# pariasm/bwd-nlkalman

Hardware: AMD Instinct MI355X
Metric: Mpix/s per frame (nlkalman-flt, 1080p sigma=20) (higher is better)
Workload: dtype f32; 1 GPU; C2: 1920x1080x3 synthetic AWGN sigma=20, FLT1 temporal (deno0 = spatial FLT1 of frame 0, bsic1=NULL), patch 8, defaults of nlkalman_default_params; parallelism=single GPU, mask_order=serial-exact, match_order=exact (the reference's hy, hx, c order)

## Files before the change

bwd-nlkalman_amd/csrc/k_frame.h:

```cpp
#pragma once
#include "nlk_common.h"

template <int CH>
__global__ void __launch_bounds__(256)
k_layout(const float* __restrict__ cur, float* __restrict__ pl_cur, const float* __restrict__ prev,
         float* __restrict__ pl_prev, const float* __restrict__ basic, float* __restrict__ pl_basic,
         uint8_t* __restrict__ rowok, float* __restrict__ acc_zero, int w, int h, int ch, int psz, int planar,
         int y0,
         uint32_t* __restrict__ zero_word,
         float* __restrict__ pl_diff) {
  const int x = blockIdx.x * blockDim.x + threadIdx.x, y = y0 + blockIdx.y;
  if (zero_word && x == 0 && blockIdx.y == 0) *zero_word = 0u;
  if (x >= w) return;
  const size_t npix = (size_t)w * h, i = (size_t)y * w + x;
  float own = 0.f;
  if constexpr (CH == 3) {
    struct __attribute__((packed, aligned(4))) P3 { float v[3]; };
    const P3 a = reinterpret_cast<const P3*>(cur)[i];
    P3 b = a, d = a;
    if (prev) b = reinterpret_cast<const P3*>(prev)[i];
    if (basic) d = reinterpret_cast<const P3*>(basic)[i];
    own = b.v[0];
#pragma unroll
    for (int c = 0; c < 3; ++c) {
      pl_cur[c * npix + i] = a.v[c];
      if (prev) pl_prev[c * npix + i] = b.v[c];
      if (basic) pl_basic[c * npix + i] = d.v[c];
      if (pl_diff) pl_diff[c * npix + i] = b.v[c] - a.v[c];
    }
  } else {
    if (prev) own = prev[i * ch];
    if (planar) {
      for (int c = 0; c < ch; ++c) {
        pl_cur[c * npix + i] = cur[i * ch + c];
        if (prev) pl_prev[c * npix + i] = prev[i * ch + c];
        if (basic) pl_basic[c * npix + i] = basic[i * ch + c];
        if (pl_diff) pl_diff[c * npix + i] = prev[i * ch + c] - cur[i * ch + c];
      }
    }
  }
  if (prev) {
#ifdef NLK_LAYOUT_ROWOK_LOADS
    uint8_t ok = (x + psz <= w);
    if (ok)
      for (int j = 0; j < psz; ++j) {
        const float v = prev[(i + j) * ch];
        if (v != v) ok = 0;
      }
    rowok[i] = ok;
#else
    const int lane = threadIdx.x & 63;
    const int xh = x + 64;
    const bool halo_nan = lane < psz - 1 && xh < w && prev[((size_t)y * w + xh) * ch] != prev[((size_t)y * w + xh) * ch];
    const uint64_t m_lo = __ballot(own != own), m_hi = __ballot(halo_nan);
    const uint64_t win = (m_lo >> lane) | (lane ? m_hi << (64 - lane) : 0ull);
    rowok[i] = (x + psz <= w) && (win & ((1ull << psz) - 1ull)) == 0ull;
#endif
  }
  if (acc_zero)
    for (int c = 0; c <= ch; ++c) acc_zero[c * npix + i] = 0.f;
}

__global__ void k_nan_cols(const uint8_t* __restrict__ rowok, uint8_t* __restrict__ valid,
                           int w, int h, int psz, int y0) {
  const int x = blockIdx.x * blockDim.x + threadIdx.x, y = y0 + blockIdx.y;
  if (x >= w) return;
  uint8_t ok = (y + psz <= h);
  if (ok)
    for (int i = 0; i < psz; ++i) ok &= rowok[(size_t)(y + i) * w + x];
  valid[(size_t)y * w + x] = ok;
}
__global__ void k_nan_cols4(const uint32_t* __restrict__ rowok, uint32_t* __restrict__ valid,
                            int w4, int h, int psz, int y0) {
  const int x = blockIdx.x * blockDim.x + threadIdx.x, y = y0 + blockIdx.y;
  if (x >= w4) return;
  uint32_t ok = (y + psz <= h) ? 0x01010101u : 0u;
  if (ok)
    for (int i = 0; i < psz; ++i) ok &= rowok[(size_t)(y + i) * w4 + x];
  valid[(size_t)y * w4 + x] = ok;
}

template <int CH>
__global__ void k_normalize(float* __restrict__ out, const float* __restrict__ acc,
                            const float* __restrict__ cur_hwc, int w, int h, int ch,
                            int y0, int y1) {
  const size_t npix = (size_t)w * h;
  for (size_t i = (size_t)y0 * w + blockIdx.x * blockDim.x + threadIdx.x;
       i < (size_t)y1 * w; i += (size_t)gridDim.x * blockDim.x) {
    if constexpr (CH == 3) {
      struct __attribute__((packed, aligned(4))) P3 { float v[3]; };
      const float a = acc[(size_t)3 * npix + i];
      P3 o;
      if (a > 1e-6f) {
#pragma unroll
        for (int c = 0; c < 3; ++c) o.v[c] = acc[(size_t)c * npix + i] / a;
      } else {
        o = reinterpret_cast<const P3*>(cur_hwc)[i];
      }
      reinterpret_cast<P3*>(out)[i] = o;
    } else {
      const float a = acc[(size_t)ch * npix + i];
      for (int c = 0; c < ch; ++c)
        out[i * ch + c] = a > 1e-6f ? acc[(size_t)c * npix + i] / a : cur_hwc[i * ch + c];
    }
  }
}

__global__ void k_add(float* __restrict__ dst, const float* __restrict__ src, size_t n) {
  for (size_t i = blockIdx.x * (size_t)blockDim.x + threadIdx.x; i < n; i += (size_t)gridDim.x * blockDim.x)
    dst[i] += src[i];
}

__global__ void k_rgb2opp(float* __restrict__ im, size_t npix) {
  const float a = 1.f / sqrtf(3.f), b = 1.f / sqrtf(2.f);
  const float c = 2.f * a * sqrtf(2.f);
  for (size_t i = blockIdx.x * (size_t)blockDim.x + threadIdx.x; i < npix;
       i += (size_t)gridDim.x * blockDim.x) {
    float* p = im + 3 * i;
    const float r = p[0], g = p[1], bl = p[2];
    p[0] = a * (r + g + bl);
// ... 85 lines not shown
```

bwd-nlkalman_amd/csrc/k_group8m.h:

```cpp
#pragma once
#include "nlk_common.h"
#include "k_commit_rows.h"
#include "k_group8.h"
#include "k_group_math.h"
#include <type_traits>

typedef float nlk_f4 __attribute__((ext_vector_type(4)));

#define NLK_G8_SST 136
#ifndef NLK_G8_CW
#define NLK_G8_CW 16
#define NLK_G8_CH 4
#endif
static inline int nlk_g8m_grid(int ntx, int nty) {
  const int nch = ((ntx + NLK_G8_CW - 1) / NLK_G8_CW) * ((nty + NLK_G8_CH - 1) / NLK_G8_CH);
  return ((nch + 7) / 8) * 8 * NLK_G8_CW * NLK_G8_CH;
}

__device__ __forceinline__ float nlk_bperm(float v, int src_lane) {
  return __int_as_float(__builtin_amdgcn_ds_bpermute(src_lane << 2, __float_as_int(v)));
}
__device__ __forceinline__ uint32_t nlk_bperm_u(uint32_t v, int src_lane) {
  return (uint32_t)__builtin_amdgcn_ds_bpermute(src_lane << 2, (int)v);
}
// ... 407 lines not shown
          constexpr bool s5_add = MODE == 1;
#endif
#pragma unroll
          for (int j = 0; j < 2; ++j) {
            const float mk = (float)((mbyte >> (2 * g4 + j)) & 1u);
#pragma unroll
            for (int q = 0; q < 4; ++q) {
              const float di = C[q][j], d = C[q][j + 2];
              if (MODE == 2) {
                S[0][q] += di;
                S[1][q] = fmaf(di, di, S[1][q]);
              }
              S[2][q] += d;
              S[3][q] = fmaf(d, d, S[3][q]);
              const float df = di - d;
              if (MODE == 2) S[4][q] = fmaf(mk * df, df, S[4][q]);
              else S[4][q] = fmaf(df, df, S[4][q]);
            }
          }
          if (s5_add) {
#pragma unroll
            for (int j = 0; j < 2; ++j) {
              const float mk = (float)((mbyte >> (2 * g4 + j)) & 1u);
#pragma unroll
              for (int q = 0; q < 4; ++q) S[5][q] = fmaf(mk, C[q][j + 2], S[5][q]);
            }
          }
        } else {
#pragma unroll
          for (int j = 0; j < 4; ++j)
#pragma unroll
            for (int q = 0; q < 4; ++q) {
              S[0][q] += C[q][j];
              S[1][q] = fmaf(C[q][j], C[q][j], S[1][q]);
            }
        }
        if (b == nb - 1) {
#if NLK_G8_S5TRACK
          if (MODE == 1 && s5_track) {
#pragma unroll
            for (int q = 0; q < 4; ++q) S[5][q] = S[2][q];
          }
          s5_track = true;
#endif
          float T[6];
#pragma unroll
          for (int a = 0; a < 6; ++a) {
            T[a] = 0.f;
            const bool used = MODE == 0 ? a < 2 : (MODE == 1 ? a >= 2 : a < 5);
            if (used) {
              const auto x = __builtin_amdgcn_permlane32_swap(__float_as_uint(S[a][0]), __float_as_uint(S[a][2]), false, false);
              const auto y = __builtin_amdgcn_permlane32_swap(__float_as_uint(S[a][1]), __float_as_uint(S[a][3]), false, false);
              const float X = __uint_as_float(x[0]) + __uint_as_float(x[1]);
              const float Y = __uint_as_float(y[0]) + __uint_as_float(y[1]);
              const auto z = __builtin_amdgcn_permlane16_swap(__float_as_uint(X), __float_as_uint(Y), false, false);
              T[a] = __uint_as_float(z[0]) + __uint_as_float(z[1]);
            }
          }
          {
            const float nx0q = g4 == 0 ? NX0[0][0] : (g4 == 1 ? NX0[1][0] : (g4 == 2 ? NX0[2][0] : NX0[3][0]));
            const float v0 = (T[3] - T[2] * T[2] * in0) * in0;
            const float v01n = T[4] * in0;
            float a, term, m;
            const float v1 = (T[1] - T[0] * T[0] * in1) * in1;
            nlk_gain<MODE, true>(v1, v0, v01n, g, s2, a, term);
            m = MODE == 2 ? 0.f : (MODE == 1 ? T[5] * ing : T[0] * in1) - nx0q;
            part_sum += term;
            const int cidx = SEPB ? 16 * (lo & 3) + 4 * g4 + (lo >> 2) : 16 * g4 + lo;
            stash[ch * SST + cidx] = a;
            stash[ch * SST + 64 + cidx] = (1 - a) * m;
          }
#pragma unroll
          for (int a = 0; a < 6; ++a)
#pragma unroll
            for (int q = 0; q < 4; ++q) S[a][q] = 0.f;
        }
      }
    };
    if (np0 == 0) pass_a(std::integral_constant<int, 0>{});
    else if (!SMO) pass_a(std::integral_constant<int, 1>{});
    else pass_a(std::integral_constant<int, 2>{});
    } else {
    float* const x0buf = stash + NSLOT * SST;
    auto sep_gain = [&](auto mode_tag, const auto& T, int ch) {
      constexpr int MODE = decltype(mode_tag)::value;
      constexpr int NS = MODE == 0 ? 2 : (MODE == 1 ? 4 : 5);
        const int oq = 2 * ((lane >> 2) & 1) + (lane >> 5), oa = (lane >> 3) & 3;
        const float nx0q = x0buf[16 * si + 4 * oq + oa];
        const int cidx = SEPB ? 16 * si + 4 * oq + oa : 16 * oq + 4 * oa + si;
        float a, term, m;
        if (MODE == 2) {
          const float v1 = (T[1] - T[0] * T[0] * in1) * in1;
          const float v0 = (T[NS > 3 ? 3 : 0] - T[NS > 2 ? 2 : 0] * T[NS > 2 ? 2 : 0] * in0) * in0;
          nlk_gain<2, true>(v1, v0, T[NS > 4 ? 4 : 0] * in0, g, s2, a, term);
          m = 0.f;
        } else if (MODE == 1) {
          const float v0 = (T[1] - T[0] * T[0] * in0) * in0;
          nlk_gain<1, true>(0.f, v0, T[NS > 2 ? 2 : 0] * in0, g, s2, a, term);
          m = (T[0] - T[NS > 3 ? 3 : 0]) * ing - nx0q;
        } else {
          const float v1 = (T[1] - T[0] * T[0] * in1) * in1;
          nlk_gain<0, true>(v1, 0.f, 0.f, g, s2, a, term);
          m = T[0] * in1 - nx0q;
        }
        part_sum += term;
        stash[ch * SST + cidx] = a;
        stash[ch * SST + 64 + cidx] = (1 - a) * m;
    };
    auto pass_a = [&](auto mode_tag) {
      constexpr int MODE = decltype(mode_tag)::value;
      constexpr bool HP = MODE != 0;
      constexpr int NS = MODE == 0 ? 2 : (MODE == 1 ? 4 : 5);
      const int nb = (k + 7) >> 3;
      if (nb == 0) return;
      const int hh = (lane >> 2) & 1, hp = lane >> 3;
      const bool odd = (lane & 1) != 0;
      const uint32_t rowx = (uint32_t)(((lane & 6) * g.w + (odd ? 4 : 0)) * 4);
      const uint32_t rowy = (uint32_t)((((lane & 6) + 1) * g.w + (odd ? 0 : 4)) * 4);
      const float sgn = hh ? -1.f : 1.f;
      float sEh[4];
#pragma unroll
      for (int i = 0; i < 4; ++i) sEh[i] = hh ? -sE[1][3 - i] : sE[0][i];
      const uint32_t e_dead = o_first + e_img;
      auto slot_offs = [&](int bb, uint32_t& oi, uint32_t& op) {
        const int ci = 8 * bb + hp, cl = min(ci, k - 1);
        const uint32_t oc = nlk_bperm_u(cl < 64 ? oreg[0] : oreg[1], cl & 63);
        const bool in_k = ci < k, valid = (oc >> 31) != 0u;
        const uint32_t o = oc & 0x7fffffffu;
        const bool live_i = MODE == 1 ? (in_k && valid) : in_k;
        oi = live_i ? o + e_img : e_dead;
        op = (in_k && valid) ? o + e_prev : e_dead;
      };
      int rows_seen = 0;
      auto row_read = [&](uint32_t off, int cc, float (&R)[8]) {
#ifdef NLK_G8_EXP_NOROWS
        if (rows_seen >= 2) { asm volatile("" : "+v"(R[0]), "+v"(R[3]), "+v"(R[5]), "+v"(R[7]) : "v"(off)); return; }
        ++rows_seen;
#endif
#ifdef NLK_G8_EXP_LDSROWS
        if (rows_seen >= 2) {
          const float* wp = smem + ((off + (uint32_t)cc * 7u + (uint32_t)(lane & 7) * 18u) % 1500u);
#pragma unroll
          for (int c = 0; c < 8; ++c) R[c] = wp[c];
          return;
        }
        ++rows_seen;
#endif
        typedef const __attribute__((address_space(1))) nlk_f4u* gp4;
        const char* bp = reinterpret_cast<const char*>(pbase);
        const uint32_t o = (off + (uint32_t)cc * (uint32_t)npix) * 4u;
        const nlk_f4u a0 = *(gp4)(bp + (size_t)(o + rowx)), a1 = *(gp4)(bp + (size_t)(o + rowy));
#pragma unroll
        for (int c = 0; c < 4; ++c) { R[c] = a0[c]; R[4 + c] = a1[c]; }
      };
      auto fold_half = [&](const float (&R)[8], float (&F)[2][4]) {
        float Z[4], S[4];
#pragma unroll
        for (int c = 0; c < 4; ++c) {
          Z[c] = odd ? R[4 + c] : R[c];
          S[c] = odd ? R[c] : R[4 + c];
        }
#pragma unroll
        for (int c = 0; c < 4; ++c) {
          const float rt = nlk_dpp<NLK_DPP_XOR1>(S[3 - c]);
          F[0][c] = Z[c] + rt;
          F[1][c] = Z[c] - rt;
        }
#define NLK_G8_FMAC_HM(i) "v_fmac_f32_dpp %" #i ", %" #i ", %8 row_half_mirror row_mask:0xf bank_mask:0xf bound_ctrl:1\n\t"
        asm("s_nop 1\n\t" NLK_G8_FMAC_HM(0) NLK_G8_FMAC_HM(1) NLK_G8_FMAC_HM(2) NLK_G8_FMAC_HM(3) NLK_G8_FMAC_HM(4)
            NLK_G8_FMAC_HM(5) NLK_G8_FMAC_HM(6) NLK_G8_FMAC_HM(7)
            : "+v"(F[0][0]), "+v"(F[0][1]), "+v"(F[0][2]), "+v"(F[0][3]), "+v"(F[1][0]), "+v"(F[1][1]), "+v"(F[1][2]),
              "+v"(F[1][3])
            : "v"(sgn));
#undef NLK_G8_FMAC_HM
      };
      auto fwd_half = [&](const float (&F)[2][4], nlk_f4 (&Y)[2]) {
        nlk_f4 T[2] = {nlk_f4{0.f, 0.f, 0.f, 0.f}, nlk_f4{0.f, 0.f, 0.f, 0.f}};
#pragma unroll
        for (int kk = 0; kk < 4; ++kk)
#pragma unroll
          for (int qc = 0; qc < 2; ++qc) T[qc] = nlk_mfma4(F[qc][kk], sE[qc][kk], T[qc]);
#pragma unroll
        for (int i = 0; i < 4; ++i)
#pragma unroll
          for (int qc = 0; qc < 2; ++qc) Y[qc] = nlk_mfma4(sEh[i], T[qc][i], Y[qc]);
      };
      nlk_f4* const x0w = reinterpret_cast<nlk_f4*>(x0buf + 16 * si + 8 * hh);
      const nlk_f4* const x0v = x0w;
      float S[NS][2][4];
#pragma unroll
      for (int a = 0; a < NS; ++a)
#pragma unroll
        for (int q = 0; q < 2; ++q)
#pragma unroll
          for (int j = 0; j < 4; ++j) S[a][q][j] = 0.f;
      float Ri[8], Rp[8];
      uint32_t oi, op, oin, opn;
      slot_offs(0, oi, op);
      const uint32_t oi0 = oi, op0 = op;
      row_read(oi, 0, Ri);
      if (HP) row_read(op, 0, Rp);
      slot_offs(1, oin, opn);
      for (int ch = 0; ch < CH; ++ch)
      for (int b = 0; b < nb; ++b) {
        const bool wrap = b + 1 == nb;
        const int chn = wrap ? min(ch + 1, CH - 1) : ch;
#ifdef NLK_G8_EXP_LDSROWS
        if (HP && b == 0) {
          float* win = stash + nlk_g8_stash_floats<CH, SEP>();
          const uint32_t back = 10u * (uint32_t)g.w + 10u;
          const uint32_t wo = (o_first > back ? o_first - back : o_first) + (uint32_t)ch * (uint32_t)npix;
          float tmp[12];
#pragma unroll
          for (int kq = 0; kq < 6; ++kq) {
            const uint32_t idx = min((uint32_t)lane + 64u * kq, 323u), r = (idx * 3641u) >> 16, cx = idx - 18u * r;
            tmp[kq] = pbase[(size_t)(e_img + wo + r * (uint32_t)g.w + cx)];
            tmp[6 + kq] = pbase[(size_t)(e_prev + wo + r * (uint32_t)g.w + cx)];
          }
#pragma unroll
          for (int kq = 0; kq < 6; ++kq) {
            win[(lane + 64 * kq) % (NLK_G8_LDS_PAD / 8)] = tmp[kq];
            win[NLK_G8_LDS_PAD / 8 + (lane + 64 * kq) % (NLK_G8_LDS_PAD / 8)] = tmp[6 + kq];
          }
          nlk_wave_lds_order();
        }
#endif
        float Fi[2][4], Fp[2][4];
        fold_half(Ri, Fi);
        if (HP) fold_half(Rp, Fp);
        uint32_t o_in = wrap ? oi0 : oin, o_pn = wrap ? op0 : opn;
        if (HP)
          asm volatile("" : "+v"(Fi[0][0]), "+v"(Fi[0][1]), "+v"(Fi[0][2]), "+v"(Fi[0][3]), "+v"(Fi[1][0]), "+v"(Fi[1][1]),
                       "+v"(Fi[1][2]), "+v"(Fi[1][3]), "+v"(Fp[0][0]), "+v"(Fp[0][1]), "+v"(Fp[0][2]), "+v"(Fp[0][3]),
                       "+v"(Fp[1][0]), "+v"(Fp[1][1]), "+v"(Fp[1][2]), "+v"(Fp[1][3]), "+v"(o_in), "+v"(o_pn));
        else
          asm volatile("" : "+v"(Fi[0][0]), "+v"(Fi[0][1]), "+v"(Fi[0][2]), "+v"(Fi[0][3]), "+v"(Fi[1][0]), "+v"(Fi[1][1]),
                       "+v"(Fi[1][2]), "+v"(Fi[1][3]), "+v"(o_in));
        __builtin_amdgcn_sched_barrier(0);
        row_read(o_in, chn, Ri);
        if (HP) row_read(o_pn, chn, Rp);
        __builtin_amdgcn_sched_barrier(0);
        slot_offs(wrap ? 1 : b + 2, oin, opn);
        nlk_f4 Yi[2], Yp[2];
        if (b == 0) {
          Yi[0] = Yi[1] = nlk_f4{0.f, 0.f, 0.f, 0.f};
          fwd_half(Fi, Yi);
          if (hp == 0) { x0w[0] = -Yi[0]; x0w[1] = -Yi[1]; }
          nlk_wave_lds_order();
          Yi[0] += x0v[0]; Yi[1] += x0v[1];
        } else {
          Yi[0] = x0v[0]; Yi[1] = x0v[1];
          fwd_half(Fi, Yi);
        }
        if (HP) {
          Yp[0] = x0v[0]; Yp[1] = x0v[1];
          fwd_half(Fp, Yp);
        }
        if constexpr (HP) {
          const uint64_t vw = b < 8 ? vbits[0] : vbits[1], gw = b < 8 ? gbits[0] : gbits[1];
          const uint32_t vch = (uint32_t)(vw >> (8 * (b & 7))) & 0xffu, gch = (uint32_t)(gw >> (8 * (b & 7))) & 0xffu;
          if constexpr (MODE == 1) {
            const bool mixed = (vch & ~gch) != 0u;
            const float mkc = (float)((~gch >> hp) & 1u);
#pragma unroll
            for (int q = 0; q < 2; ++q)
#pragma unroll
              for (int j = 0; j < 4; ++j) {
                const float di = Yi[q][j], d = Yp[q][j];
                const float df = di - d;
                if (b == 0) {
                  S[0][q][j] = d;
                  S[1][q][j] = d * d;
                  S[2][q][j] = df * df;
                } else {
                  S[0][q][j] += d;
                  S[1][q][j] = fmaf(d, d, S[1][q][j]);
                  S[2][q][j] = fmaf(df, df, S[2][q][j]);
                }
              }
            if (mixed) {
#pragma unroll
              for (int q = 0; q < 2; ++q)
#pragma unroll
                for (int j = 0; j < 4; ++j) S[NS > 3 ? 3 : 0][q][j] = fmaf(mkc, Yp[q][j], S[NS > 3 ? 3 : 0][q][j]);
            }
          } else {
            const float mk = (float)((vch >> hp) & 1u);
#pragma unroll
            for (int q = 0; q < 2; ++q)
#pragma unroll
              for (int j = 0; j < 4; ++j) {
                const float di = Yi[q][j], d = Yp[q][j];
                S[0][q][j] += di;
                S[1][q][j] = fmaf(di, di, S[1][q][j]);
                S[NS > 2 ? 2 : 0][q][j] += d;
                S[NS > 3 ? 3 : 0][q][j] = fmaf(d, d, S[NS > 3 ? 3 : 0][q][j]);
                const float df = di - d;
                S[NS > 4 ? 4 : 0][q][j] = fmaf(mk * df, df, S[NS > 4 ? 4 : 0][q][j]);
              }
          }
        } else {
#pragma unroll
          for (int q = 0; q < 2; ++q)
#pragma unroll
            for (int j = 0; j < 4; ++j) {
              S[0][q][j] += Yi[q][j];
              S[1][q][j] = fmaf(Yi[q][j], Yi[q][j], S[1][q][j]);
            }
        }
        if (wrap) {
          float T[NS];
          const bool hi8 = (lane & 8) != 0;
#pragma unroll
          for (int a = 0; a < NS; ++a) {
            float Z[4], W[2];
#pragma unroll
            for (int j = 0; j < 4; ++j) {
              const auto z = __builtin_amdgcn_permlane32_swap(__float_as_uint(S[a][0][j]), __float_as_uint(S[a][1][j]), false, false);
              Z[j] = __uint_as_float(z[0]) + __uint_as_float(z[1]);
            }
#pragma unroll
            for (int j = 0; j < 2; ++j) {
              const auto z = __builtin_amdgcn_permlane16_swap(__float_as_uint(Z[j]), __float_as_uint(Z[j + 2]), false, false);
              W[j] = __uint_as_float(z[0]) + __uint_as_float(z[1]);
            }
            const float send = hi8 ? W[0] : W[1], keep = hi8 ? W[1] : W[0];
            T[a] = keep + nlk_dpp<NLK_DPP_ROR8>(send);
            if (!(MODE == 1 && a < 3)) {
#pragma unroll
              for (int q = 0; q < 2; ++q)
#pragma unroll
                for (int j = 0; j < 4; ++j) S[a][q][j] = 0.f;
            }
          }
          sep_gain(mode_tag, T, ch);
        }
      }
    };
    if (np0 == 0) pass_a(std::integral_constant<int, 0>{});
    else if (!SMO) pass_a(std::integral_constant<int, 1>{});
    else pass_a(std::integral_constant<int, 2>{});
    }

    nlk_wave_lds_order();
#ifndef NLK_G8_M5
#define NLK_G8_M5 1
#endif
    constexpr bool M5 = NLK_G8_M5 && SEPB && CH == 3;
    constexpr int MPS = G16 ? 16 : (M5 ? 5 : 4);
    constexpr int NPX = M5 ? 5 : 4;
    const bool wlane = SEPB && spl == 3;
    const int bchc = G16 ? 0 : (M5 ? (wlane ? min(g4, CH - 1) : spl) : min(bch, CH - 1));
// ... 292 lines not shown
```

bwd-nlkalman_amd/csrc/nlk_hip.hip:

```cpp
#include <math.h>
#include <time.h>

#include <algorithm>
#include <mutex>
#include <vector>

namespace nlk_host12 {
#define NLK_HD static inline
#include "k_dct12.h"
#undef NLK_HD
}

#include "k_commit.h"
#include "k_frame.h"
#include "k_match.h"
#include "nlk_internal.h"

char nlk_g_err[512] = "";

namespace {

std::mutex g_live_mu;
std::vector<nlk_ctx*> g_live;

// ... 296 lines not shown
  if (!c) return NLK_EINVAL;
  NLK_USE_DEVICE(c);
  if (h) HIPCHK(c, hipHostFree(h));
  return NLK_OK;
}
int nlk_sync(nlk_ctx* c) {
  if (!c) return NLK_EINVAL;
  NLK_USE_DEVICE(c);
  HIPCHK(c, hipStreamSynchronize(c->stream));
  return NLK_OK;
}

int nlk_dev_rgb2opp(nlk_ctx* c, float* im, int w, int h, int ch) {
  int rc = check_images(c, im, im, w, h, ch);
  if (rc) return rc;
  NLK_USE_DEVICE(c);
  if (ch != 3) return NLK_OK;
  hipLaunchKernelGGL(k_rgb2opp, dim3(2048), dim3(256), 0, c->stream, im, (size_t)w * h);
  HIPCHK(c, hipGetLastError());
  return NLK_OK;
}

int nlk_dev_opp2rgb(nlk_ctx* c, float* im, int w, int h, int ch) {
  int rc = check_images(c, im, im, w, h, ch);
  if (rc) return rc;
  NLK_USE_DEVICE(c);
  if (ch != 3) return NLK_OK;
  hipLaunchKernelGGL(k_opp2rgb, dim3(2048), dim3(256), 0, c->stream, im, (size_t)w * h);
  HIPCHK(c, hipGetLastError());
  return NLK_OK;
}

int nlk_dev_warp_bicubic(nlk_ctx* c, float* imw, const float* im, const float* of,
                         const float* msk, int w, int h, int ch) {
  int rc = check_images(c, imw, im, w, h, ch);
  if (rc) return rc;
  NLK_USE_DEVICE(c);
  if (!of) return fail(c, NLK_EINVAL, "null flow");
  auto kern = ch == 3 ? k_warp_bicubic<3> : (ch == 1 ? k_warp_bicubic<1> : k_warp_bicubic<0>);
  hipLaunchKernelGGL(kern, dim3((w + 127) / 128, h), dim3(128), 0, c->stream, imw,
                     im, of, msk, w, h, ch);
  HIPCHK(c, hipGetLastError());
  return NLK_OK;
}

struct NlkPlan {
  NlkGeom g{};
  const float *img_cur = nullptr, *img_prev = nullptr, *img_basic = nullptr, *img_match = nullptr;
  const float* img_diff = nullptr;
  NlkTile tl{}, tw{};
  size_t lds = 0, lds_w = 0;
  int maxm = 0, maxm_w = 0;
  bool wide = false;
  bool wide0_zeroed = false;
  bool generic = false;
};

static NlkRecView view_rows(nlk_ctx* c, const NlkGeom& g, hipStream_t stream, int r0, int band) {
  const size_t t0 = (size_t)r0 * g.ngx;
  NlkRecView v;
  v.stream = stream;
  v.topk = (uint32_t*)c->topk.p + t0 * g.kmax;
  v.tinfo = (NlkTarget*)c->tinfo.p + t0;
  v.gcoords = (uint32_t*)c->gcoords.p + t0 * g.gstride;
  v.marks = (c->marks_ext ? c->marks_ext : (uint64_t*)c->marks.p) + t0;
  v.wide = (uint32_t*)c->wide.p + t0 + band;
  return v;
}

static NlkGeom band_geom(const NlkGeom& g, int r0, int rows) {
  NlkGeom b = g;
  b.oy = g.oy + r0 * g.step;
  b.ngy = rows;
  return b;
}

static int layout_rows(nlk_ctx* c, const float* cur, const float* prev, const float* basic, float* acc_zero, int w,
                       int h, int ch, int psz, int y0, int y1, int v0, int v1, uint32_t* zero_word = nullptr) {
  const size_t img_floats = (size_t)w * h * ch;
  float* const slab = (float*)c->planes.p;
  if (y1 > y0)
    hipLaunchKernelGGL(ch == 3 ? k_layout<3> : k_layout<0>, dim3((w + 255) / 256, y1 - y0), dim3(256), 0, c->stream, cur, slab, prev,
                       slab + img_floats, basic, slab + 2 * img_floats, (uint8_t*)c->rowok.p, acc_zero, w, h, ch, psz,
                       1, y0, zero_word, (c->layout_diff && prev) ? slab + 3 * img_floats : nullptr);
  if (prev && v1 > v0) {
    if (w % 4 == 0)
      hipLaunchKernelGGL(k_nan_cols4, dim3((w / 4 + 255) / 256, v1 - v0), dim3(256), 0, c->stream,
                         (const uint32_t*)c->rowok.p, (uint32_t*)c->vmap.p, w / 4, h, psz, v0);
    else
      hipLaunchKernelGGL(k_nan_cols, dim3((w + 255) / 256, v1 - v0), dim3(256), 0, c->stream, (const uint8_t*)c->rowok.p,
                         (uint8_t*)c->vmap.p, w, h, psz, v0);
  }
  HIPCHK(c, hipGetLastError());
  return NLK_OK;
}

static int plan_frame(nlk_ctx* c, NlkPlan& pl, const float* cur, const float* prev, const float* basic, int w,
                      int h, int ch, float sigma, const struct nlkalman_params* P, int oy, int ngy,
                      int smoother, int nbands, float* acc_zero = nullptr, bool do_layout = true) {
  int rc = check_images(c, cur, cur, w, h, ch);
  if (rc) return rc;
  if (!P) return fail(c, NLK_EINVAL, "null parameters");
  NLK_USE_DEVICE(c);
  c->lazy_ngx = c->lazy_ngy = 0;
  c->lazy_dst = nullptr;
  NlkGeom& g = pl.g;
  g.w = w; g.h = h; g.ch = ch;
  g.psz = P->patch_sz;
  if (g.psz < 2 || g.psz > 32 || ch * g.psz * g.psz > 4096)
    return fail(c, NLK_EUNSUP, "patch size %d with %d channels not supported (2..32, ch * psz^2 <= 4096)", g.psz, ch);
  g.step = g.psz / 2;
  g.p2 = g.psz * g.psz;
  g.E = g.p2 * ch;
  if (w < g.psz || h < g.psz) return fail(c, NLK_EINVAL, "image smaller than a patch");
  g.ngx = (w - g.psz) / g.step + 1;
  g.oy = oy;
  g.ngy = ngy;
  if (oy < 0 || ngy < 1 || oy + (ngy - 1) * g.step + g.psz > h)
    return fail(c, NLK_EINVAL, "target rows [%d + j*%d, j < %d) leave the %d-row strip", oy,
                g.step, ngy, h);
  g.wsz_x = P->search_sz_x; g.wsz_t = P->search_sz_t;
  g.npx = P->npatches_x; g.npt = P->npatches_t; g.ntagg = P->npatches_tagg;
  if (g.wsz_x < 0 || g.wsz_t < 0 || g.ntagg < 0)
    return fail(c, NLK_EINVAL, "negative search radius or group size (call nlkalman_default_params first)");
  g.have_prev = prev != nullptr;
  g.have_basic = basic != nullptr;
  g.smoother = smoother != 0;
  g.sigma2 = sigma * sigma;
  g.beta_x = P->beta_x; g.beta_t = P->beta_t;
  const int wmax = g.smoother ? g.wsz_t : (g.have_prev ? max(g.wsz_x, g.wsz_t) : g.wsz_x);
  const int wmark = (g.smoother || g.have_prev) ? g.wsz_t : g.wsz_x;
  g.R = wmark / g.step;
  const int ncand = (2 * wmax + 1) * (2 * wmax + 1);
  pl.generic = !(g.psz == 4 || g.psz == 6 || g.psz == 8 || g.psz == 10 || g.psz == 12 || g.psz == 16) ||
               !(ch == 1 || ch == 3) || ncand > 64 * 16 || nlk_set(c->sw.generic_match);
  g.kmax = max(max(g.npx, g.npt), 1);
  const int ngrid = g.ngx * g.ngy;
  const int npix = w * h;
  const int ntagg_alloc = max(g.ntagg, 1);
  g.gstride = ntagg_alloc;

  mark(c, 0);
  {
    const size_t img_floats = (size_t)npix * ch;
    c->layout_diff = g.smoother && prev != nullptr;
    if ((rc = reserve(c, c->planes, sizeof(float) * img_floats * (c->layout_diff ? 4 : (basic ? 3 : (prev ? 2 : 1)))))) return rc;
    pl.img_diff = c->layout_diff ? (const float*)c->planes.p + 3 * img_floats : nullptr;
    c->p_diff = pl.img_diff;
    pl.img_cur = (const float*)c->planes.p;
    pl.img_prev = prev ? pl.img_cur + img_floats : nullptr;
    pl.img_basic = basic ? pl.img_cur + 2 * img_floats : nullptr;
    if (prev && ((rc = reserve(c, c->rowok, npix)) || (rc = reserve(c, c->vmap, npix)))) return rc;
    if ((rc = reserve(c, c->wide, sizeof(uint32_t) * ((size_t)ngrid + nbands)))) return rc;
    if (do_layout) {
      int rc2 = layout_rows(c, cur, prev, basic, acc_zero, w, h, ch, g.psz, 0, h, 0, h, (uint32_t*)c->wide.p);
      if (rc2) return rc2;
      pl.wide0_zeroed = true;
    }
  }
  if ((rc = upload_tables(c, g.psz))) return rc;
  if ((rc = reserve(c, c->topk, sizeof(uint32_t) * (size_t)ngrid * g.kmax)) ||
      (rc = reserve(c, c->tinfo, sizeof(NlkTarget) * (size_t)ngrid)) ||
      (rc = reserve(c, c->gcoords, sizeof(uint32_t) * (size_t)ngrid * ntagg_alloc)) ||
      (rc = reserve(c, c->marks, sizeof(uint64_t) * (size_t)ngrid)) ||
      (rc = reserve(c, c->active, (size_t)ngrid)))
    return rc;
  mark(c, 1);

  pl.img_match = basic ? pl.img_basic : pl.img_cur;
  NlkTile& tl = pl.tl;
  const bool small_grid = (size_t)((g.ngx + 7) / 8) * ((g.ngy + 3) / 4) < 576;
  tl.tgx = nlk_or(c->sw.mtx, small_grid ? 4 : 8);
  tl.tgy = nlk_or(c->sw.mty, small_grid ? 2 : 4);
  tl.threads = NLK_BM_THREADS;
  tl.bx = 4;
  {
    const int halo0 = (g.smoother || g.have_prev) ? g.wsz_t : g.wsz_x;
    const bool tiles84 = tl.tgx == 8 && tl.tgy == 4 && (nlk_set(c->sw.match_block) || !small_grid);
    const int rounds0 = ((2 * halo0 + 1) * (2 * halo0 + 1) + 63) / 64;
    if (nlk_or(c->sw.match_wg8, 0) != 0 && g.psz <= 8 && tiles84) { tl.threads = 512; tl.tgy = 8; }
    else if (nlk_or(c->sw.match_bx2, 1) != 0 && tiles84 && g.psz >= 8 && (rounds0 <= 2 || (g.psz == 8 && rounds0 <= 7))) {
      tl.threads = 512;
      tl.bx = 2;
    }
  }
  tl.ntx = (g.ngx + tl.tgx - 1) / tl.tgx;
  tl.block = nlk_set(c->sw.match_noblock) ? 0 : (nlk_set(c->sw.match_block) ? 1 : !small_grid);
  tl.order = (nlk_or(c->sw.match_order, 0) == 1 && g.psz == 8) ? 1 : 0;
  tl.halo = (g.smoother || g.have_prev) ? g.wsz_t : g.wsz_x;
  {
    const int need = (tl.tgx - 1) * g.step + 2 * tl.halo + g.psz;
    const int wdom = 2 * tl.halo + 1;
    tl.rwp = need + ((wdom - need) % 32 + 32) % 32;
  }
  tl.rh_max = (tl.tgy - 1) * g.step + 2 * tl.halo + g.psz;
  tl.ksel_max = g.kmax;
  auto tile_lds = [&]() {
    return sizeof(float) * ((size_t)ch * tl.rwp * tl.rh_max + 1 + (size_t)(tl.threads / 64) * (3 * tl.ksel_max + ntagg_alloc));
  };
  pl.lds = tile_lds();
  if (pl.lds > 160 * 1024 && tl.threads > NLK_BM_THREADS && tl.tgy == 4) {
    tl.threads = NLK_BM_THREADS;
    tl.bx = 4;
    pl.lds = tile_lds();
  }
  if (pl.lds > 160 * 1024) pl.generic = true;
  pl.wide = !pl.generic && g.have_prev && !g.smoother && g.wsz_x > g.wsz_t;
  const int wdom = 2 * tl.halo + 1;
  pl.maxm = (wdom * wdom + 63) / 64;
  if (pl.wide) {
    NlkTile& tw = pl.tw;
    tw = tl;
    const int need = 2 * g.wsz_x + g.psz, ww = 2 * g.wsz_x + 1;
    tw.halo = g.wsz_x;
    tw.rwp = need + ((ww - need) % 32 + 32) % 32;
    tw.rh_max = need;
    const size_t per_wave = (((size_t)ch * tw.rwp * tw.rh_max + 1) & ~(size_t)1) +
                            ((3 * (size_t)tw.ksel_max + ntagg_alloc + 1) & ~(size_t)1);
    pl.lds_w = sizeof(float) * NLK_BM_WAVES * per_wave;
    if (pl.lds_w > 160 * 1024) { pl.generic = true; pl.wide = false; }
    pl.maxm_w = (ncand + 63) / 64;
  }
  c->p_match = pl.img_match; c->p_cur = pl.img_cur; c->p_prev = pl.img_prev;
  c->last = g;
  c->have_last = true;
  return NLK_OK;
}

static int match_rows(nlk_ctx* c, const NlkPlan& pl, hipStream_t stream, int r0, int rows, int band) {
// ... 542 lines not shown
```

bwd-nlkalman_amd/csrc/nlk_internal.h:

```cpp
#pragma once
#include <hip/hip_runtime.h>
#include <stdarg.h>
#include <stdint.h>
#include <stdio.h>
#include <stdlib.h>
#include <string.h>

#include "../../include/nlk_hip.h"
#include "nlk_common.h"

struct NlkTvMail;
struct NlkTile;
struct NlkGTile;

struct NlkBuf {
  void* p = nullptr;
  size_t cap = 0;
  void* base = nullptr;
};

struct NlkRecView {
  hipStream_t stream = nullptr;
  uint32_t* topk = nullptr;
  NlkTarget* tinfo = nullptr;
  uint32_t* gcoords = nullptr;
  uint64_t* marks = nullptr;
  uint32_t* wide = nullptr;
  const uint32_t* chase_planes = nullptr;
  uint64_t* chase_words = nullptr;
  const uint32_t* chase_gen = nullptr;
  int chase_reach = 0, chase_row0 = 0, chase_rows = 0;
};

#define NLK_UNSET (-2147483647 - 1)
#define NLK_SWITCH_LIST(X)                                                                                   \
  X(deterministic, "NLK_DETERMINISTIC") X(generic_group, "NLK_GENERIC_GROUP") X(group_packed, "NLK_GROUP_PACKED") \
  X(group_dpp, "NLK_GROUP_DPP") X(group_sep, "NLK_GROUP_SEP") X(group_ilp, "NLK_GROUP_ILP") X(generic_match, "NLK_GENERIC_MATCH") X(mtx, "NLK_MTX") X(mty, "NLK_MTY")    \
  X(match_wg8, "NLK_MATCH_WG8") X(match_bx2, "NLK_MATCH_BX2") X(match_block, "NLK_MATCH_BLOCK")              \
  X(match_noblock, "NLK_MATCH_NOBLOCK") X(match_order, "NLK_MATCH_ORDER") X(commit_wave, "NLK_COMMIT_WAVE") X(commit_lds, "NLK_COMMIT_LDS")    \
  X(commit_band, "NLK_COMMIT_BAND") X(no_chase, "NLK_NO_CHASE") X(chase_test_skip0, "NLK_CHASE_TEST_SKIP0") X(bands, "NLK_BANDS") X(host_bands, "NLK_HOST_BANDS")                    \
  X(host_trace, "NLK_HOST_TRACE") X(gtx, "NLK_GTX") X(gty, "NLK_GTY") X(g8_tail, "NLK_G8_TAIL")              \
  X(g8_single, "NLK_G8_SINGLE") X(tv_wg_pixels, "NLK_TV_WG_PIXELS") X(tv_unblocked, "NLK_TV_UNBLOCKED")      \
  X(tv_batch, "NLK_TV_BATCH") X(tv_mid, "NLK_TV_MID") X(tv_shape, "NLK_TV_SHAPE") X(tv_deep, "NLK_TV_DEEP")  \
  X(tv_inline, "NLK_TV_INLINE") X(tv_wg_full, "NLK_TV_WG_FULL") X(tv_look, "NLK_TV_LOOK") X(tv_look2, "NLK_TV_LOOK2") X(tv_trace, "NLK_TV_TRACE")
struct NlkSwitches {
#define NLK_X(field, name) int field = NLK_UNSET;
  NLK_SWITCH_LIST(NLK_X)
#undef NLK_X
  void load() {
#define NLK_X(field, name) { const char* e_ = getenv(name); field = e_ ? atoi(e_) : NLK_UNSET; }
    NLK_SWITCH_LIST(NLK_X)
#undef NLK_X
    if (const char* e_ = getenv("NLK_MATCH_ORDER")) match_order = (!strcmp(e_, "block") || atoi(e_) == 1) ? 1 : 0;
  }
};
static inline bool nlk_set(int v) { return v != NLK_UNSET; }
static inline int nlk_or(int v, int dflt) { return v != NLK_UNSET ? v : dflt; }

struct nlk_ctx {
  int device = 0;
  NlkSwitches sw;
  hipStream_t own_stream = nullptr;
  hipStream_t stream = nullptr;
  hipStream_t aux_stream = nullptr;
  hipEvent_t sync_ev[8] = {};
  NlkRecView rv;
  bool chase_on = false;
  int chase_row0 = 0, chase_rows = 0;
  int lazy_ngx = 0, lazy_ngy = 0;
  unsigned char* lazy_dst = nullptr;
  uint64_t* marks_ext = nullptr;
  float* strip_acc = nullptr;
  char err[512] = "";
  NlkBuf planes;
  NlkBuf rowok, vmap, topk, tinfo, gcoords, marks, active, acc, tabs, wide;
  NlkBuf skew;
  NlkBuf chase;
  NlkBuf ms;
  NlkBuf lz3;
  void* lz3_old[16] = {};
  int lz3_nold = 0;
  NlkBuf tv;
  NlkBuf bm;
  NlkBuf sqd;
  NlkBuf sig;
  NlkBuf curve;
  NlkBuf ssim;
  NlkBuf sure;
  NlkBuf nlf;
  float* nlf_host = nullptr;
  NlkBuf slab, tflag;
  NlkBuf hw_cur, hw_prev, hw_basic, hw_out;
  hipStream_t up_stream = nullptr, dn_stream = nullptr;
  hipEvent_t band_ev[5][8] = {};
  bool deterministic = false;
  NlkTvMail* tv_host = nullptr;
  unsigned tv_seq = 0;
  int tabs_psz = 0;
  NlkGeom last{};
  bool have_last = false;
  const float *p_match = nullptr, *p_cur = nullptr, *p_prev = nullptr;
  const float* p_diff = nullptr;
  bool layout_diff = false;
  static constexpr int NEV = 7, MAXSETS = 512;
  bool profiling = false;
  bool recording = false;
  bool set_open = false;
  unsigned set_seen = 0;
  hipEvent_t* ev = nullptr;
  int nsets = 0;
  nlk_timings tm{};
};

extern char nlk_g_err[512];

static inline int fail(nlk_ctx* c, int code, const char* fmt, ...) {
  char msg[512];
  va_list ap;
  va_start(ap, fmt);
  vsnprintf(msg, sizeof msg, fmt, ap);
  va_end(ap);
  snprintf(nlk_g_err, sizeof nlk_g_err, "%s", msg);
  if (c) snprintf(c->err, sizeof c->err, "%s", msg);
  return code;
}

#define HIPCHK(ctx, call)                                                         \
  do {                                                                            \
    hipError_t e_ = (call);                                                       \
    if (e_ != hipSuccess)                                                         \
      return fail(ctx, NLK_EHIP, "%s failed: %s (%s:%d)", #call,                  \
                  hipGetErrorString(e_), __FILE__, __LINE__);                     \
  } while (0)

#define NLK_USE_DEVICE(ctx) HIPCHK(ctx, hipSetDevice((ctx)->device))

static inline int reserve(nlk_ctx* c, NlkBuf& b, size_t bytes) {
  if (bytes <= b.cap) return NLK_OK;
  if (b.p) HIPCHK(c, hipFree(b.base ? b.base : b.p));
  b.p = b.base = nullptr;
  b.cap = 0;
  static const bool guard = getenv("NLK_DEBUG_GUARD") != nullptr;
  if (guard) {
    const size_t page = (size_t)2 << 20, used = (bytes + 255) & ~(size_t)255, want = (used + page - 1) / page * page;
    if (hipMalloc(&b.base, want) != hipSuccess) return fail(c, NLK_ENOMEM, "hipMalloc of %zu bytes failed", want);
    b.p = (char*)b.base + (want - used);
    b.cap = bytes;
    return NLK_OK;
  }
  const size_t want = bytes + bytes / 8 + 256;
  if (hipMalloc(&b.p, want) != hipSuccess)
    return fail(c, NLK_ENOMEM, "hipMalloc of %zu bytes failed", want);
  b.cap = want;
  return NLK_OK;
}

int nlk_launch_group8(nlk_ctx* c, const NlkGeom& g, const float* img, const float* cur, const float* prev,
                      float* acc, const uint8_t* active);
int nlk_launch_groupp_a(nlk_ctx* c, const NlkGeom& g, const float* img, const float* cur, const float* prev,
                        float* acc, const uint8_t* active);
int nlk_launch_groupp_b(nlk_ctx* c, const NlkGeom& g, const float* img, const float* cur, const float* prev,
                        float* acc, const uint8_t* active);
int nlk_launch_groupp_c(nlk_ctx* c, const NlkGeom& g, const float* img, const float* cur, const float* prev,
                        float* acc, const uint8_t* active);
int nlk_launch_group_generic(nlk_ctx* c, const NlkGeom& g, const float* img, const float* cur,
                             const float* prev, float* acc, const uint8_t* active);
int nlk_launch_group_any(nlk_ctx* c, const NlkGeom& g, const float* img, const float* cur, const float* prev,
                         float* acc, const uint8_t* active);
int nlk_launch_match(nlk_ctx* c, const NlkGeom& g, const NlkTile& tl, size_t lds, const float* img,
                     int maxm, bool wide);
int nlk_launch_match_generic(nlk_ctx* c, const NlkGeom& g, const float* img);
```

bwd-nlkalman_amd/csrc/tu_group8.hip:

```cpp
#include "k_gather.h"
#include "k_group8.h"
#include "k_group8m.h"
#include "nlk_internal.h"

const void* nlk_group8m_ilp_kernel(int ch, bool smoother, int sep);

namespace {

template <int CH, bool SMO>
int launch_group8_t(nlk_ctx* c, const NlkGeom& g, const float* img, const float* cur,
                    const float* prev, float* acc, const uint8_t* active) {
  constexpr int PSZ = 8;
  const bool mfma = !nlk_set(c->sw.group_dpp);
  const int sep_default = g.ch == 1 ? 6 : (!g.smoother && prev) ? 6 : (g.ntagg < 4 ? 0 : 2);
  int sep = mfma ? nlk_or(c->sw.group_sep, sep_default) : 0;
  if (sep != 0 && sep != 6) sep = 2;
  if (mfma) {
    const float* lo = (const float*)c->planes.p;
    const float* hi = lo + c->planes.cap / sizeof(float);
    const bool inside = img >= lo && img < hi && cur >= lo && cur < hi && (!prev || (prev >= lo && prev < hi));
    if (!inside || c->planes.cap >= ((size_t)1 << 32)) {
      if (c->rv.chase_words) return fail(c, NLK_EINVAL, "internal: mask replay handed to a group kernel that cannot run it");
      return nlk_launch_groupp_a(c, g, img, cur, prev, acc, active);
    }
  }
  if (mfma && SMO && prev && !(c->p_diff && cur == c->p_cur && prev == c->p_prev)) {
    if (c->rv.chase_words) return fail(c, NLK_EINVAL, "internal: mask replay handed to a group kernel that cannot run it");
    return nlk_launch_groupp_a(c, g, img, cur, prev, acc, active);
  }
  if (c->rv.chase_words && (!mfma || c->deterministic))
    return fail(c, NLK_EINVAL, "internal: mask replay handed to a group kernel that cannot run it");
  if (c->deterministic && !mfma)
    return fail(c, NLK_EUNSUP, "deterministic aggregation is not available in the NLK_GROUP_DPP variant");
  const bool split = c->deterministic && g.have_prev && !g.smoother && g.wsz_x > g.wsz_t;
  auto shape = [&](int pass) {
    NlkGTile tl{};
    tl.pbase = (const float*)c->planes.p;
    tl.diff = (SMO && prev) ? c->p_diff : nullptr;
    tl.split = split;
    tl.far = pass;
    tl.chase = c->rv.chase_words ? c->rv.chase_reach : 0;
    tl.chase_test_skip0 = nlk_set(c->sw.chase_test_skip0);
    tl.chase_gen = c->rv.chase_gen;
    tl.chase_row0 = c->rv.chase_row0;
    tl.chase_rows = c->rv.chase_rows;
    tl.chase_planes = c->rv.chase_planes;
    tl.chase_words = c->rv.chase_words;
    tl.wmax = (g.smoother || g.have_prev) ? g.wsz_t : g.wsz_x;
    if (pass == 1) tl.wmax = g.wsz_x;
    auto tiles_with = [&](int t) { return (size_t)((g.ngx + t - 1) / t) * g.ngy; };
    const int tgx_fill = tiles_with(3) >= 30000 ? 3 : (tiles_with(2) >= 2560 ? 2 : 1);
    const bool wide_full = mfma && tl.wmax > 6 && tgx_fill == 3 && pass == 0;
    tl.tgx = nlk_or(c->sw.gtx, wide_full ? (CH == 1 ? 3 : 2) : min(tgx_fill, tl.wmax > 6 ? 2 : 4));
    tl.tgy = nlk_or(c->sw.gty, (mfma && tgx_fill == 3 && tl.wmax <= 6) || wide_full ? 2 : 1);
    tl.ntx = (g.ngx + tl.tgx - 1) / tl.tgx;
    tl.nty = (g.ngy + tl.tgy - 1) / tl.tgy;
    tl.nty_full = tl.nty;
    tl.single = 0;
    if (mfma && (tl.tgy > 1 || tl.tgx > 1) && !c->deterministic) {
      int tail = tl.tgy == 1 ? 0 : nlk_or(c->sw.g8_tail, (2560 + tl.ntx / 2) / tl.ntx);
      int single = nlk_or(c->sw.g8_single, (2880 + g.ngx / 2) / g.ngx);
      single = max(0, min(single, g.ngy / 8));
      tail = max(0, min(tail, g.ngy / 4));
      tl.single = single;
      const int rows = g.ngy - tl.single;
      tl.nty_full = (rows - tail) / tl.tgy;
      tl.nty = tl.nty_full + (rows - tl.nty_full * tl.tgy);
    }
    tl.nmain = mfma ? nlk_g8m_grid(tl.ntx, tl.nty) : 0;
    const int rw_max = (tl.tgx - 1) * g.step + 2 * tl.wmax + g.psz;
    tl.rh_max = (tl.tgy - 1) * g.step + 2 * tl.wmax + g.psz;
    if (mfma && sep != 0 && CH > 1) {
      tl.rwp = rw_max + ((2 - rw_max) % 4 + 4) % 4;
      tl.plane = tl.rwp * tl.rh_max;
      tl.plane += ((8 - tl.plane) % 16 + 16) % 16;
    } else if (mfma) {
      tl.rwp = rw_max + ((4 - rw_max) % 8 + 8) % 8;
      tl.plane = tl.rwp * tl.rh_max;
      tl.plane += ((16 - tl.plane) % 32 + 32) % 32;
    } else {
      tl.rwp = rw_max | 1;
      tl.plane = tl.rwp * tl.rh_max;
    }
    return tl;
  };
  const int npass = split ? 2 : 1;
  NlkGTile tls[2] = {shape(0), shape(split ? 1 : 0)};
  size_t slab_at[2] = {0, 0}, flag_at[2] = {0, 0}, cnt_at[2] = {0, 0};
  if (c->deterministic) {
    size_t need = 0, nflag = 0, ncnt = 0;
    for (int pass = 0; pass < npass; ++pass) {
      const size_t ntiles = (size_t)tls[pass].ntx * tls[pass].nty;
      slab_at[pass] = need; flag_at[pass] = nflag; cnt_at[pass] = ncnt;
      need += ntiles * (CH + 1) * tls[pass].plane;
      nflag += ntiles;
      ncnt += 1 + (size_t)tls[pass].nty;
    }
    const size_t cnt_off = (nflag + 15) & ~(size_t)15, cnt_bytes = sizeof(int) * ncnt;
    int rc;
    if ((rc = reserve(c, c->slab, sizeof(float) * need)) || (rc = reserve(c, c->tflag, cnt_off + cnt_bytes))) return rc;
    HIPCHK(c, hipMemsetAsync((uint8_t*)c->tflag.p + cnt_off, 0, cnt_bytes, c->rv.stream));
    for (int pass = 0; pass < npass; ++pass) {
      tls[pass].slab = (float*)c->slab.p + slab_at[pass];
      tls[pass].tflag = (uint8_t*)c->tflag.p + flag_at[pass];
      tls[pass].tcount = (int*)((uint8_t*)c->tflag.p + cnt_off) + cnt_at[pass];
    }
  }
  for (int pass = 0; pass < npass; ++pass) {
    const NlkGTile& tl = tls[pass];
#ifndef NLK_G8_LDS_PAD
#define NLK_G8_LDS_PAD 0
#endif
    const size_t stash = !mfma ? 0 : sep == 0 ? nlk_g8_stash_floats<CH, 0>() : sep == 2 ? nlk_g8_stash_floats<CH, 2>() : nlk_g8_stash_floats<CH, 6>();
    const size_t lds = sizeof(float) * ((size_t)(CH + 1) * tl.plane + stash) + NLK_G8_LDS_PAD;
    if (lds > 160 * 1024) return fail(c, NLK_EUNSUP, "aggregation tile needs %zu bytes of LDS", lds);
    void (*kern)(const float*, const float*, const float*, const uint8_t*, NlkGeom, NlkGTile,
                 const uint32_t*, const NlkTarget*, const uint32_t*, const uint8_t*, const float*,
                 const float*, float*);
    kern = !mfma ? k_group8<CH, SMO> : sep == 0 ? k_group8m<CH, SMO, 0> : sep == 2 ? k_group8m<CH, SMO, 2> : k_group8m<CH, SMO, 6>;
    if (mfma && nlk_or(c->sw.group_ilp, 1) != 0)
      if (const void* k2 = nlk_group8m_ilp_kernel(CH, SMO, sep)) kern = reinterpret_cast<decltype(kern)>(const_cast<void*>(k2));
// ... 27 lines not shown
```

Baseline: 2272 Mpix/s.

## Precompute prev-minus-basic difference plane for filter-mode separable group pass

For the non-smoother filter path with 8x8 patches and the separable mode, the layout kernel now also writes a planar prev-minus-basic difference image. The group kernel's MODE 1 path then transforms that difference directly instead of transforming the image patch and subtracting the transformed prev patch. Dead slots point at a zeroed tail region that is memset once and cached in the context. This removes per-patch transform work in the aggregation kernel. In exchange the layout pass writes an extra full plane, the planes buffer grows, and there is extra bookkeeping for the cached zero region.

```diff
diff --git a/bwd-nlkalman_amd/csrc/k_frame.h b/bwd-nlkalman_amd/csrc/k_frame.h
--- a/bwd-nlkalman_amd/csrc/k_frame.h
+++ b/bwd-nlkalman_amd/csrc/k_frame.h
@@ -8,7 +8,8 @@
          uint8_t* __restrict__ rowok, float* __restrict__ acc_zero, int w, int h, int ch, int psz, int planar,
          int y0,
          uint32_t* __restrict__ zero_word,
-         float* __restrict__ pl_diff) {
+         float* __restrict__ pl_diff,
+         int diff_stat) {
   const int x = blockIdx.x * blockDim.x + threadIdx.x, y = y0 + blockIdx.y;
   if (zero_word && x == 0 && blockIdx.y == 0) *zero_word = 0u;
   if (x >= w) return;
@@ -26,7 +27,7 @@
       pl_cur[c * npix + i] = a.v[c];
       if (prev) pl_prev[c * npix + i] = b.v[c];
       if (basic) pl_basic[c * npix + i] = d.v[c];
-      if (pl_diff) pl_diff[c * npix + i] = b.v[c] - a.v[c];
+      if (pl_diff) pl_diff[c * npix + i] = b.v[c] - (diff_stat ? d.v[c] : a.v[c]);
     }
   } else {
     if (prev) own = prev[i * ch];
@@ -35,7 +36,7 @@
         pl_cur[c * npix + i] = cur[i * ch + c];
         if (prev) pl_prev[c * npix + i] = prev[i * ch + c];
         if (basic) pl_basic[c * npix + i] = basic[i * ch + c];
-        if (pl_diff) pl_diff[c * npix + i] = prev[i * ch + c] - cur[i * ch + c];
+        if (pl_diff) pl_diff[c * npix + i] = prev[i * ch + c] - ((diff_stat && basic) ? basic : cur)[i * ch + c];
       }
     }
   }
diff --git a/bwd-nlkalman_amd/csrc/k_group8m.h b/bwd-nlkalman_amd/csrc/k_group8m.h
--- a/bwd-nlkalman_amd/csrc/k_group8m.h
+++ b/bwd-nlkalman_amd/csrc/k_group8m.h
@@ -513,6 +513,8 @@
     else pass_a(std::integral_constant<int, 2>{});
     } else {
     float* const x0buf = stash + NSLOT * SST;
+    const uint32_t e_diff = tl.diff ? (uint32_t)(tl.diff - pbase) : e_img;
+    const uint32_t e_zero = e_diff + (uint32_t)CH * (uint32_t)npix;
     auto sep_gain = [&](auto mode_tag, const auto& T, int ch) {
       constexpr int MODE = decltype(mode_tag)::value;
       constexpr int NS = MODE == 0 ? 2 : (MODE == 1 ? 4 : 5);
@@ -552,15 +554,23 @@
       float sEh[4];
 #pragma unroll
       for (int i = 0; i < 4; ++i) sEh[i] = hh ? -sE[1][3 - i] : sE[0][i];
-      const uint32_t e_dead = o_first + e_img;
+      uint32_t o_fv = o_first;
+      if constexpr (MODE == 1) {
+        const int fv = vbits[0] ? __builtin_ctzll(vbits[0]) : __builtin_ctzll(vbits[1]);
+        const int ofv = vbits[0] ? __builtin_amdgcn_readlane((int)oreg[0], fv) : __builtin_amdgcn_readlane((int)oreg[1], fv);
+        o_fv = (uint32_t)ofv & 0x7fffffffu;
+      }
+      const uint32_t e_first = MODE == 1 ? e_diff : e_img;
+      const uint32_t e_dead_i = MODE == 1 ? e_zero : o_first + e_img;
+      const uint32_t e_dead_p = MODE == 1 ? o_fv + e_prev : o_first + e_img;
       auto slot_offs = [&](int bb, uint32_t& oi, uint32_t& op) {
         const int ci = 8 * bb + hp, cl = min(ci, k - 1);
         const uint32_t oc = nlk_bperm_u(cl < 64 ? oreg[0] : oreg[1], cl & 63);
         const bool in_k = ci < k, valid = (oc >> 31) != 0u;
         const uint32_t o = oc & 0x7fffffffu;
         const bool live_i = MODE == 1 ? (in_k && valid) : in_k;
-        oi = live_i ? o + e_img : e_dead;
-        op = (in_k && valid) ? o + e_prev : e_dead;
+        oi = live_i ? o + e_first : e_dead_i;
+        op = (in_k && valid) ? o + e_prev : e_dead_p;
       };
       int rows_seen = 0;
       auto row_read = [&](uint32_t off, int cc, float (&R)[8]) {
@@ -673,19 +683,34 @@
         __builtin_amdgcn_sched_barrier(0);
         slot_offs(wrap ? 1 : b + 2, oin, opn);
         nlk_f4 Yi[2], Yp[2];
-        if (b == 0) {
+        if constexpr (MODE == 1) {
           Yi[0] = Yi[1] = nlk_f4{0.f, 0.f, 0.f, 0.f};
           fwd_half(Fi, Yi);
-          if (hp == 0) { x0w[0] = -Yi[0]; x0w[1] = -Yi[1]; }
-          nlk_wave_lds_order();
-          Yi[0] += x0v[0]; Yi[1] += x0v[1];
+          if (b == 0) {
+            Yp[0] = Yp[1] = nlk_f4{0.f, 0.f, 0.f, 0.f};
+            fwd_half(Fp, Yp);
+            if (hp == 0) { x0w[0] = -Yp[0]; x0w[1] = -Yp[1]; }
+            nlk_wave_lds_order();
+            Yp[0] += x0v[0]; Yp[1] += x0v[1];
+          } else {
+            Yp[0] = x0v[0]; Yp[1] = x0v[1];
+            fwd_half(Fp, Yp);
+          }
         } else {
-          Yi[0] = x0v[0]; Yi[1] = x0v[1];
-          fwd_half(Fi, Yi);
-        }
-        if (HP) {
-          Yp[0] = x0v[0]; Yp[1] = x0v[1];
-          fwd_half(Fp, Yp);
+          if (b == 0) {
+            Yi[0] = Yi[1] = nlk_f4{0.f, 0.f, 0.f, 0.f};
+            fwd_half(Fi, Yi);
+            if (hp == 0) { x0w[0] = -Yi[0]; x0w[1] = -Yi[1]; }
+            nlk_wave_lds_order();
+            Yi[0] += x0v[0]; Yi[1] += x0v[1];
+          } else {
+            Yi[0] = x0v[0]; Yi[1] = x0v[1];
+            fwd_half(Fi, Yi);
+          }
+          if (HP) {
+            Yp[0] = x0v[0]; Yp[1] = x0v[1];
+            fwd_half(Fp, Yp);
+          }
         }
         if constexpr (HP) {
           const uint64_t vw = b < 8 ? vbits[0] : vbits[1], gw = b < 8 ? gbits[0] : gbits[1];
@@ -697,8 +722,7 @@
             for (int q = 0; q < 2; ++q)
 #pragma unroll
               for (int j = 0; j < 4; ++j) {
-                const float di = Yi[q][j], d = Yp[q][j];
-                const float df = di - d;
+                const float df = Yi[q][j], d = Yp[q][j];
                 if (b == 0) {
                   S[0][q][j] = d;
                   S[1][q][j] = d * d;
diff --git a/bwd-nlkalman_amd/csrc/nlk_hip.hip b/bwd-nlkalman_amd/csrc/nlk_hip.hip
--- a/bwd-nlkalman_amd/csrc/nlk_hip.hip
+++ b/bwd-nlkalman_amd/csrc/nlk_hip.hip
@@ -402,7 +402,7 @@
   if (y1 > y0)
     hipLaunchKernelGGL(ch == 3 ? k_layout<3> : k_layout<0>, dim3((w + 255) / 256, y1 - y0), dim3(256), 0, c->stream, cur, slab, prev,
                        slab + img_floats, basic, slab + 2 * img_floats, (uint8_t*)c->rowok.p, acc_zero, w, h, ch, psz,
-                       1, y0, zero_word, (c->layout_diff && prev) ? slab + 3 * img_floats : nullptr);
+                       1, y0, zero_word, (c->layout_diff && prev) ? slab + 3 * img_floats : nullptr, c->layout_diff == 2);
   if (prev && v1 > v0) {
     if (w % 4 == 0)
       hipLaunchKernelGGL(k_nan_cols4, dim3((w / 4 + 255) / 256, v1 - v0), dim3(256), 0, c->stream,
@@ -463,8 +463,23 @@
   mark(c, 0);
   {
     const size_t img_floats = (size_t)npix * ch;
-    c->layout_diff = g.smoother && prev != nullptr;
-    if ((rc = reserve(c, c->planes, sizeof(float) * img_floats * (c->layout_diff ? 4 : (basic ? 3 : (prev ? 2 : 1)))))) return rc;
+    const bool fdiff = !g.smoother && prev != nullptr && g.psz == 8 && (ch == 1 || ch == 3) &&
+                       (nlk_group8_sep(c, ch, false, true, g.ntagg) & 4) != 0;
+    c->layout_diff = (g.smoother && prev != nullptr) ? 1 : (fdiff ? 2 : 0);
+    const size_t zero_at = 4 * img_floats, zero_floats = fdiff ? (size_t)(ch - 1) * npix + (size_t)8 * w : 0;
+    const size_t laid = img_floats * (c->layout_diff ? 4 : (basic ? 3 : (prev ? 2 : 1)));
+    const size_t cap0 = c->planes.cap;
+    if ((rc = reserve(c, c->planes, sizeof(float) * (laid + zero_floats)))) return rc;
+    if (c->planes.cap != cap0) c->zero_slab = nullptr;
+    if (fdiff) {
+      if (c->zero_slab != c->planes.p || c->zero_at != zero_at || c->zero_npix != (size_t)npix || c->zero_w != w || c->zero_ch != ch) {
+        for (int cc = 0; cc < ch; ++cc)
+          HIPCHK(c, hipMemsetAsync((float*)c->planes.p + zero_at + (size_t)cc * npix, 0, sizeof(float) * 8 * w, c->stream));
+        c->zero_slab = c->planes.p; c->zero_at = zero_at; c->zero_npix = (size_t)npix; c->zero_w = w; c->zero_ch = ch;
+      }
+    } else if (c->zero_slab && laid > c->zero_at) {
+      c->zero_slab = nullptr;
+    }
     pl.img_diff = c->layout_diff ? (const float*)c->planes.p + 3 * img_floats : nullptr;
     c->p_diff = pl.img_diff;
     pl.img_cur = (const float*)c->planes.p;
diff --git a/bwd-nlkalman_amd/csrc/nlk_internal.h b/bwd-nlkalman_amd/csrc/nlk_internal.h
--- a/bwd-nlkalman_amd/csrc/nlk_internal.h
+++ b/bwd-nlkalman_amd/csrc/nlk_internal.h
@@ -101,7 +101,10 @@
   bool have_last = false;
   const float *p_match = nullptr, *p_cur = nullptr, *p_prev = nullptr;
   const float* p_diff = nullptr;
-  bool layout_diff = false;
+  int layout_diff = 0;
+  const void* zero_slab = nullptr;
+  size_t zero_at = 0, zero_npix = 0;
+  int zero_w = 0, zero_ch = 0;
   static constexpr int NEV = 7, MAXSETS = 512;
   bool profiling = false;
   bool recording = false;
@@ -155,6 +158,13 @@
   return NLK_OK;
 }
 
+static inline int nlk_group8_sep(const nlk_ctx* c, int ch, bool smoother, bool have_prev, int ntagg) {
+  if (nlk_set(c->sw.group_dpp)) return 0;
+  const int sep_default = ch == 1 ? 6 : (!smoother && have_prev) ? 6 : (ntagg < 4 ? 0 : 2);
+  const int sep = nlk_or(c->sw.group_sep, sep_default);
+  return (sep != 0 && sep != 6) ? 2 : sep;
+}
+
 int nlk_launch_group8(nlk_ctx* c, const NlkGeom& g, const float* img, const float* cur, const float* prev,
                       float* acc, const uint8_t* active);
 int nlk_launch_groupp_a(nlk_ctx* c, const NlkGeom& g, const float* img, const float* cur, const float* prev,
diff --git a/bwd-nlkalman_amd/csrc/tu_group8.hip b/bwd-nlkalman_amd/csrc/tu_group8.hip
--- a/bwd-nlkalman_amd/csrc/tu_group8.hip
+++ b/bwd-nlkalman_amd/csrc/tu_group8.hip
@@ -12,9 +12,7 @@
                     const float* prev, float* acc, const uint8_t* active) {
   constexpr int PSZ = 8;
   const bool mfma = !nlk_set(c->sw.group_dpp);
-  const int sep_default = g.ch == 1 ? 6 : (!g.smoother && prev) ? 6 : (g.ntagg < 4 ? 0 : 2);
-  int sep = mfma ? nlk_or(c->sw.group_sep, sep_default) : 0;
-  if (sep != 0 && sep != 6) sep = 2;
+  const int sep = nlk_group8_sep(c, g.ch, g.smoother, prev != nullptr, g.ntagg);
   if (mfma) {
     const float* lo = (const float*)c->planes.p;
     const float* hi = lo + c->planes.cap / sizeof(float);
@@ -28,6 +26,9 @@
     if (c->rv.chase_words) return fail(c, NLK_EINVAL, "internal: mask replay handed to a group kernel that cannot run it");
     return nlk_launch_groupp_a(c, g, img, cur, prev, acc, active);
   }
+  const bool fdiff = mfma && !SMO && prev && (sep & 4);
+  if (fdiff && !(c->p_diff && c->layout_diff == 2 && img == c->p_match && prev == c->p_prev))
+    return fail(c, NLK_EINVAL, "internal: a filter call's separable pass A without its difference plane");
   if (c->rv.chase_words && (!mfma || c->deterministic))
     return fail(c, NLK_EINVAL, "internal: mask replay handed to a group kernel that cannot run it");
   if (c->deterministic && !mfma)
@@ -36,7 +37,7 @@
   auto shape = [&](int pass) {
     NlkGTile tl{};
     tl.pbase = (const float*)c->planes.p;
-    tl.diff = (SMO && prev) ? c->p_diff : nullptr;
+    tl.diff = ((SMO && prev) || fdiff) ? c->p_diff : nullptr;
     tl.split = split;
     tl.far = pass;
     tl.chase = c->rv.chase_words ? c->rv.chase_reach : 0;
```

Result: no change. 2282 Mpix/s, median of 6 (+0.5%).
